# HipGraph/iSpLib

Measured on AMD Instinct MI355X. Metric: edges_aggregated_per_sec, higher is better.
Workload: dtype f32

## Files before the change

include/isplib_hip.h:

```cpp
#ifndef ISPLIB_HIP_H
#define ISPLIB_HIP_H

#include <stddef.h>
#include <stdint.h>

#ifdef __cplusplus
extern "C" {
#endif

#define ISPLIB_HIP_ABI_VERSION 1
#define ISPLIB_MAX_SLICES 4096

#define ISPLIB_VOP_COPY_RHS 0x2
#define ISPLIB_ROP_NOOP     0x00
#define ISPLIB_SOP_COPY     0x100
#define ISPLIB_VSC_MUL      0x1000
#define ISPLIB_VSC_MEAN     0x3000
#define ISPLIB_AOP_ADD      0x10000
#define ISPLIB_AOP_MAX      0x20000
#define ISPLIB_AOP_MIN      0x30000
#define ISPLIB_MSG_SPMM_SUM  (ISPLIB_VOP_COPY_RHS | ISPLIB_ROP_NOOP | ISPLIB_SOP_COPY | ISPLIB_VSC_MUL  | ISPLIB_AOP_ADD)
#define ISPLIB_MSG_SPMM_MEAN (ISPLIB_VOP_COPY_RHS | ISPLIB_ROP_NOOP | ISPLIB_SOP_COPY | ISPLIB_VSC_MEAN | ISPLIB_AOP_ADD)
#define ISPLIB_MSG_SPMM_MAX  (ISPLIB_VOP_COPY_RHS | ISPLIB_ROP_NOOP | ISPLIB_SOP_COPY | ISPLIB_VSC_MUL  | ISPLIB_AOP_MAX)
#define ISPLIB_MSG_SPMM_MIN  (ISPLIB_VOP_COPY_RHS | ISPLIB_ROP_NOOP | ISPLIB_SOP_COPY | ISPLIB_VSC_MUL  | ISPLIB_AOP_MIN)
// ... 133 lines not shown
typedef struct isplib_stream_plan {
   int64_t rows, cols;
   int32_t slices, gens, waves_per_gen, rows_per_wave, streams , chunk ;
   int64_t n_steps, n_parts, n_hub;
   const int32_t *words;
   const float   *vals;
   const int64_t *wave_step_off;
   const int32_t *wave_row;
   const int32_t *wave_part;
   const int32_t *hub_row;
   const int32_t *hub_off;
   const int32_t *perm;
} isplib_stream_plan;
int  isplib_stream_plan_build_hip(int64_t m, int64_t n, int64_t nnz, const int64_t *rowptr, const int64_t *col,
                                  const float *val, int streams, int slices, int chunk, int waves_per_gen,
                                  isplib_stream_plan *out , void *stream);
int  isplib_stream_plan_set_values_hip(isplib_stream_plan *plan, const float *val , void *stream);
void isplib_stream_plan_free(isplib_stream_plan *plan);
int    isplib_spmm_stream_geometry(int streams, int *rows_per_wave , int *waves_resident );
int    isplib_suggest_stream(int64_t m, int64_t n, int64_t nnz, int64_t k, int *streams, int *slices, int *chunk);
int    isplib_suggest_stream_weighted(int64_t m, int64_t n, int64_t nnz, int64_t k, int weighted, int *streams, int *slices, int *chunk);
int    isplib_spmm_stream_minmax_geometry(int streams , int *rows_per_wave , int *waves_resident );
int    isplib_suggest_stream_minmax(int64_t m, int64_t n, int64_t nnz, int64_t k, int *streams, int *slices, int *chunk);
int    isplib_stream_plan_build_minmax_hip(int64_t m, int64_t n, int64_t nnz, const int64_t *rowptr, const int64_t *col,
                                           const float *val, int streams, int slices, int chunk, int waves_per_gen,
                                           isplib_stream_plan *out , void *stream);
size_t isplib_spmm_stream_minmax_workspace_bytes(const isplib_stream_plan *plan);
int    fusedMM_csr_stream_minmax_hip(int32_t imessage , int64_t m, int64_t n, int64_t k,
                                     int64_t nnz, const int64_t *pntrb, const int64_t *pntre,
                                     const isplib_stream_plan *plan ,
                                     const float *y, int64_t ldy, float *z, int64_t ldz, int64_t *z_arg,
                                     void *workspace, size_t workspace_bytes, void *stream);
size_t isplib_spmm_stream_workspace_bytes(const isplib_stream_plan *plan);
int    fusedMM_csr_stream_hip(int32_t imessage , int64_t m, int64_t n, int64_t k,
                              int64_t nnz, const int64_t *pntrb, const int64_t *pntre,
                              const isplib_stream_plan *plan ,
                              const float *y, int64_t ldy, float *z, int64_t ldz,
                              void *workspace, size_t workspace_bytes,
                              const isplib_epilogue *epilogue , void *stream);

int    isplib_fusedmm_stream_geometry(int streams, int *rows_per_wave , int *waves_resident );
int    isplib_suggest_fusedmm_stream(int32_t imessage, int64_t m, int64_t n, int64_t nnz, int64_t k, int *streams, int *slices, int *chunk);
int    isplib_stream_plan_build_fusedmm_hip(int64_t m, int64_t n, int64_t nnz, const int64_t *rowptr, const int64_t *col,
                                            int streams, int slices, int chunk, int waves_per_gen,
                                            isplib_stream_plan *out , void *stream);
int    fusedMM_csr_udef_stream_hip(int32_t imessage, int64_t m, int64_t n, int64_t k, int64_t nnz,
                                   const int64_t *pntrb, const int64_t *pntre, const isplib_stream_plan *plan ,
                                   const float *x , int64_t ldx, const float *y , int64_t ldy,
                                   float *z , int64_t ldz, int sop_udef , float sop_param,
                                   void *workspace, size_t workspace_bytes, void *stream);

int    fusedMM_csr_ordered_hip(int32_t imessage, int64_t m, int64_t n, int64_t k, int64_t nnz, const float *val,
                               const int64_t *indx, const int64_t *pntrb, const int64_t *pntre,
                               const int32_t *row_order , const float *y, int64_t ldy, float *z,
                               int64_t ldz, int64_t *z_arg, void *stream);

int    isplib_plain_panels(int64_t n, int64_t ldy);

size_t isplib_community_order_workspace_bytes(int64_t m, int64_t nnz);
int    isplib_community_order_hip(int64_t m, int64_t nnz, const int64_t *rowptr, const int64_t *col, int rounds, int seed,
                                  int32_t *order, int32_t *labels , int *rounds_run ,
                                  void *workspace, size_t workspace_bytes, void *stream);
int    isplib_order_locality_hip(int64_t m, int64_t nnz, const int64_t *rowptr, const int64_t *col, const int32_t *order,
                                 int64_t window, double *share , void *workspace ,
                                 size_t workspace_bytes, void *stream);

// ... 64 lines not shown
```

isplib_amd/cabi.py:

```python
from __future__ import annotations

import ctypes
import os
from typing import Optional

import torch

from . import _lib

MSG_SPMM_SUM = 0x2 | 0x00 | 0x100 | 0x1000 | 0x10000
MSG_SPMM_MEAN = 0x2 | 0x00 | 0x100 | 0x3000 | 0x10000
MSG_SPMM_MAX = 0x2 | 0x00 | 0x100 | 0x1000 | 0x20000
MSG_SPMM_MIN = 0x2 | 0x00 | 0x100 | 0x1000 | 0x30000
MESSAGE = {"sum": MSG_SPMM_SUM, "add": MSG_SPMM_SUM, "mean": MSG_SPMM_MEAN, "max": MSG_SPMM_MAX, "min": MSG_SPMM_MIN}

SUCCESS, FAIL, NOT_ENOUGH_MEM, NO_OPT_IMPL, HIP_ERROR = 0, 1, -1, 128, 256
UNDEFINED_USER_FUNCTION = 64

VOP = {"copy_lhs": 0x1, "copy_rhs": 0x2, "add": 0x3, "subl": 0x4, "subr": 0x5, "max": 0x6, "min": 0x7, "udef": 0xF}
ROP = {"noop": 0x00, "dot": 0x10, "add_lhs": 0x20, "add_rhs": 0x30, "norml": 0x40, "normr": 0x50, "udef": 0xF0}
SOP = {"noop": 0x000, "copy": 0x100, "udef": 0xF00}
VSC = {"noop": 0x0000, "mul": 0x1000, "add": 0x2000, "mean": 0x3000, "udef": 0xF000}
AOP = {"add": 0x10000, "max": 0x20000, "min": 0x30000, "udef": 0xF0000}
SOP_UDEF = {"none": 0, "sigmoid": 1, "one_minus_sigmoid": 2, "tdist": 3, "scale": 4, "exp": 5, "leaky_exp": 6}
PATTERNS = {
    "spmm": (MSG_SPMM_SUM, "none"),
    "sigmoid_embedding": (VOP["copy_rhs"] | ROP["dot"] | SOP["udef"] | VSC["mul"] | AOP["add"], "sigmoid"),
    "tdist_embedding": (VOP["subr"] | ROP["normr"] | SOP["udef"] | VSC["mul"] | AOP["add"], "tdist"),
    "attention_sum": (VOP["copy_rhs"] | ROP["dot"] | SOP["udef"] | VSC["mul"] | AOP["add"], "leaky_exp"),
}

EXPORTS = (
    "isplib_hip_abi_version", "isplib_hip_last_error", "isplib_hip_set_empty_row", "isplib_hip_get_empty_row", "fusedMM_csr_hip", "performDummySpMM_hip",
    "isplib_spmm_minmax_bw_hip", "isplib_sddmm_csr_hip", "isplib_csr_row_ids_hip",
    "isplib_csr2csc_workspace_bytes", "isplib_csr2csc_hip",
    "isplib_spmm_slices_bytes", "isplib_spmm_slices_build_hip", "isplib_spmm_sliced_workspace_bytes",
    "fusedMM_csr_sliced_hip", "fusedMM_csr_sliced_phase_hip", "isplib_hip_tune",
    "isplib_spmm_tasks_workspace_bytes", "fusedMM_csr_tasks_hip",
    "isplib_spmm_tasks_plan_workspace_bytes", "isplib_spmm_tasks_count_hip", "isplib_spmm_tasks_fill_hip",
    "isplib_sddmm_csr_tasks_hip", "fusedMM_csr_tasks_epilogue_hip", "fusedMM_csr_udef_hip", "fusedMM_csr_udef_tasks_hip", "isplib_pack_indices_hip",
    "isplib_suggest_slices", "isplib_graph_create", "isplib_graph_set_slices", "isplib_graph_set_values", "isplib_graph_spmm", "isplib_graph_spmm_backward",
    "isplib_graph_destroy", "isplib_suggest_slices_whole_rows", "isplib_graph_sddmm",
    "fusedMM_csr_stream_hip", "isplib_spmm_stream_workspace_bytes", "isplib_spmm_stream_geometry", "isplib_suggest_stream", "isplib_suggest_stream_weighted", "isplib_stream_plan_build_hip", "isplib_stream_plan_build_minmax_hip", "fusedMM_csr_stream_minmax_hip", "isplib_spmm_stream_minmax_geometry", "isplib_suggest_stream_minmax", "isplib_spmm_stream_minmax_workspace_bytes", "isplib_stream_plan_set_values_hip", "isplib_stream_plan_free", "isplib_spmm_minmax_bw_det_hip", "isplib_spmm_minmax_bw_workspace_bytes", "isplib_scatter_rows_det_hip",
    "isplib_fusedmm_stream_geometry", "isplib_suggest_fusedmm_stream", "isplib_stream_plan_build_fusedmm_hip", "fusedMM_csr_udef_stream_hip",
    "isplib_row_scale_hip", "isplib_masked_scale_colsum_hip", "isplib_masked_scale_colsum_workspace_bytes",
    "fusedMM_csr_ordered_hip", "isplib_community_order_hip", "isplib_community_order_workspace_bytes", "isplib_order_locality_hip",
    "isplib_graph_set_row_order", "isplib_plain_panels",
)

EXP_EXPORTS = ("fusedMM_csr_sweep_hip", "isplib_spmm_sweep_workspace_bytes", "isplib_spmm_sweep_resident_waves",
               "fusedMM_csr_hybrid_hip", "isplib_spmm_hybrid_geometry", "isplib_spmm_hybrid_workspace_bytes", "isplib_sddmm_stream_hip",
               "isplib_hip_tune_experimental")

_i64, _f32, _vp, _i32 = ctypes.c_int64, ctypes.c_float, ctypes.c_void_p, ctypes.c_int32


class Epilogue(ctypes.Structure):
    _fields_ = [("row_scale", ctypes.c_void_p), ("self", ctypes.c_void_p), ("ld_self", ctypes.c_int64),
                ("bias", ctypes.c_void_p), ("relu", ctypes.c_int)]


class TaskPlanInfo(ctypes.Structure):
    _fields_ = [("n_tasks", ctypes.c_int64), ("lane_off", ctypes.c_int64 * 9), ("slices", ctypes.c_int32),
                ("chunk", ctypes.c_int32), ("short_row", ctypes.c_int32), ("reserved", ctypes.c_int32)]


class SweepPlanStruct(ctypes.Structure):
    _fields_ = [("rows", ctypes.c_int64), ("slices", ctypes.c_int32), ("gens", ctypes.c_int32),
                ("waves_per_gen", ctypes.c_int32), ("rows_per_wave", ctypes.c_int32), ("n_tasks", ctypes.c_int64),
                ("n_parts", ctypes.c_int64), ("n_hub", ctypes.c_int64), ("wave_row", ctypes.c_void_p),
                ("wave_part", ctypes.c_void_p), ("wave_task_off", ctypes.c_void_p), ("task_b", ctypes.c_void_p),
                ("task_meta", ctypes.c_void_p), ("hub_row", ctypes.c_void_p), ("hub_off", ctypes.c_void_p)]


class StreamPlanStruct(ctypes.Structure):
    _fields_ = [("rows", ctypes.c_int64), ("cols", ctypes.c_int64), ("slices", ctypes.c_int32), ("gens", ctypes.c_int32),
# ... 128 lines not shown
        L.isplib_spmm_stream_minmax_geometry.argtypes = [ctypes.c_int, ctypes.POINTER(ctypes.c_int), ctypes.POINTER(ctypes.c_int)]
        L.isplib_suggest_stream_minmax.restype = ctypes.c_int
        L.isplib_suggest_stream_minmax.argtypes = [_i64, _i64, _i64, _i64, ctypes.POINTER(ctypes.c_int), ctypes.POINTER(ctypes.c_int), ctypes.POINTER(ctypes.c_int)]
        L.isplib_spmm_stream_minmax_workspace_bytes.restype = ctypes.c_size_t
        L.isplib_spmm_stream_minmax_workspace_bytes.argtypes = [ctypes.POINTER(StreamPlanStruct)]
        L.fusedMM_csr_stream_minmax_hip.restype = ctypes.c_int
        L.fusedMM_csr_stream_minmax_hip.argtypes = [_i32, _i64, _i64, _i64, _i64, _vp, _vp, ctypes.POINTER(StreamPlanStruct), _vp, _i64,
                                                    _vp, _i64, _vp, _vp, ctypes.c_size_t, _vp]
        L.isplib_stream_plan_set_values_hip.restype = ctypes.c_int
        L.isplib_stream_plan_set_values_hip.argtypes = [ctypes.POINTER(StreamPlanStruct), _vp, _vp]
        L.isplib_stream_plan_free.restype = None
        L.isplib_stream_plan_free.argtypes = [ctypes.POINTER(StreamPlanStruct)]
        L.isplib_community_order_workspace_bytes.restype = ctypes.c_size_t
        L.isplib_community_order_workspace_bytes.argtypes = [_i64, _i64]
        L.isplib_community_order_hip.restype = ctypes.c_int
        L.isplib_community_order_hip.argtypes = [_i64, _i64, _vp, _vp, ctypes.c_int, ctypes.c_int, _vp, _vp, ctypes.POINTER(ctypes.c_int), _vp,
                                                 ctypes.c_size_t, _vp]
        L.isplib_order_locality_hip.restype = ctypes.c_int
        L.isplib_order_locality_hip.argtypes = [_i64, _i64, _vp, _vp, _vp, _i64, ctypes.POINTER(ctypes.c_double), _vp, ctypes.c_size_t, _vp]
        L.isplib_graph_set_row_order.restype = ctypes.c_int
        L.isplib_graph_set_row_order.argtypes = [_vp, _vp, _vp]
        L.fusedMM_csr_ordered_hip.restype = ctypes.c_int
        L.fusedMM_csr_ordered_hip.argtypes = [_i32, _i64, _i64, _i64, _i64, _vp, _vp, _vp, _vp, _vp, _vp, _i64, _vp, _i64, _vp, _vp]
        L.isplib_plain_panels.restype = ctypes.c_int
        L.isplib_plain_panels.argtypes = [_i64, _i64]
        L.isplib_suggest_stream.restype = ctypes.c_int
        L.isplib_suggest_stream.argtypes = [_i64, _i64, _i64, _i64, ctypes.POINTER(ctypes.c_int), ctypes.POINTER(ctypes.c_int), ctypes.POINTER(ctypes.c_int)]
        L.isplib_suggest_stream_weighted.restype = ctypes.c_int
        L.isplib_suggest_stream_weighted.argtypes = [_i64, _i64, _i64, _i64, ctypes.c_int, ctypes.POINTER(ctypes.c_int), ctypes.POINTER(ctypes.c_int), ctypes.POINTER(ctypes.c_int)]
        L.isplib_spmm_stream_geometry.restype = ctypes.c_int
        L.isplib_spmm_stream_geometry.argtypes = [ctypes.c_int, ctypes.POINTER(ctypes.c_int), ctypes.POINTER(ctypes.c_int)]
        L.isplib_spmm_stream_workspace_bytes.restype = ctypes.c_size_t
        L.isplib_spmm_stream_workspace_bytes.argtypes = [ctypes.POINTER(StreamPlanStruct)]
        L.fusedMM_csr_stream_hip.restype = ctypes.c_int
        L.fusedMM_csr_stream_hip.argtypes = [_i32, _i64, _i64, _i64, _i64, _vp, _vp, ctypes.POINTER(StreamPlanStruct), _vp, _i64,
                                             _vp, _i64, _vp, ctypes.c_size_t, ctypes.POINTER(Epilogue), _vp]
        _sigs_set = True
    return L


_exp = None


def exp_lib() -> ctypes.CDLL:
    global _exp
    if _exp is None:
        lib()
        path = os.path.join(os.path.dirname(_lib.CABI_PATH), "libisplib_hip_exp.so")
        if not os.path.exists(path):
            raise ImportError(f"isplib_amd: '{os.path.basename(path)}' not found; build it with `make -C isplib_amd/csrc`")
        L = ctypes.CDLL(path, mode=ctypes.RTLD_GLOBAL)
        L.isplib_hip_tune_experimental.restype = ctypes.c_int
        L.isplib_hip_tune_experimental.argtypes = [ctypes.c_int, ctypes.c_int]
        L.isplib_spmm_hybrid_geometry.restype = ctypes.c_int
        L.isplib_spmm_hybrid_geometry.argtypes = [ctypes.c_int] + [ctypes.POINTER(ctypes.c_int)] * 4
        L.isplib_spmm_hybrid_workspace_bytes.restype = ctypes.c_size_t
        L.isplib_spmm_hybrid_workspace_bytes.argtypes = [ctypes.POINTER(HybridPlanStruct)]
        L.fusedMM_csr_hybrid_hip.restype = ctypes.c_int
        L.fusedMM_csr_hybrid_hip.argtypes = [_i32, _i64, _i64, _i64, _i64, _vp, _vp, ctypes.POINTER(HybridPlanStruct), _vp, _i64, _vp, _i64,
                                             _vp, ctypes.c_size_t, _vp, _vp]
        L.isplib_sddmm_stream_hip.restype = ctypes.c_int
        L.isplib_sddmm_stream_hip.argtypes = [_i64, _i64, _i64, _i64, _vp, _vp, ctypes.POINTER(StreamPlanStruct), _vp, _i64, _vp, _i64,
                                              ctypes.c_int, _vp, _vp]
        L.isplib_spmm_sweep_resident_waves.restype = ctypes.c_int
        L.isplib_spmm_sweep_resident_waves.argtypes = [_i32, _i64, ctypes.c_int]
        L.isplib_spmm_sweep_workspace_bytes.restype = ctypes.c_size_t
# ... 585 lines not shown
        ep = Epilogue(None if row_scale is None else row_scale.data_ptr(), None if self_term is None else self_term.data_ptr(),
                      k if self_term is None else self_term.stride(0), None if bias is None else bias.data_ptr(), int(bool(relu)))
    fusedMM_csr_stream_hip(MESSAGE[reduce], rowptr, nnz, plan, y, out, workspace, ep)
    return out


def fusedMM_csr_stream_minmax_hip(imessage: int, rowptr, nnz: int, plan, y, z, z_arg=None, workspace=None, check: bool = True) -> int:
    assert y.is_cuda and y.dtype == torch.float32 and y.dim() == 2 and y.stride(1) == 1
    m, n, k = rowptr.numel() - 1, y.size(0), y.size(1)
    rp = rowptr.data_ptr()
    ps = plan.struct()
    with torch.cuda.device(y.device):
        st = lib().fusedMM_csr_stream_minmax_hip(int(imessage), m, n, k, int(nnz), ctypes.c_void_p(rp), ctypes.c_void_p(rp + 8),
                                                 ctypes.byref(ps), _ptr(y), y.stride(0) if n > 1 else max(k, y.stride(0)), _ptr(z),
                                                 z.stride(0) if m > 1 else max(k, z.stride(0)), _ptr(z_arg), _ptr(workspace),
                                                 0 if workspace is None else workspace.numel(), _stream(y.device))
    if check:
        _check(st, "fusedMM_csr_stream_minmax_hip")
    return st


def spmm_stream_minmax(rowptr, nnz: int, plan, y, reduce: str = "max", workspace=None, want_arg: bool = True):
    rowptr = _dev(rowptr, "rowptr", torch.int64)
    y = y.contiguous()
    m, k = rowptr.numel() - 1, y.size(1)
    out = torch.empty((m, k), dtype=torch.float32, device=y.device)
    arg = torch.empty((m, k), dtype=torch.int64, device=y.device) if want_arg else None
    if workspace is None:
        workspace = plan.workspace(minmax=True)
    fusedMM_csr_stream_minmax_hip(MESSAGE[reduce], rowptr, nnz, plan, y, out, arg, workspace)
    return out, arg


def suggest_stream_minmax(m: int, n: int, nnz: int, k: int):
    st, sl, ch = ctypes.c_int(0), ctypes.c_int(0), ctypes.c_int(0)
    if not lib().isplib_suggest_stream_minmax(int(m), int(n), int(nnz), int(k), ctypes.byref(st), ctypes.byref(sl), ctypes.byref(ch)):
        return None
    return st.value, sl.value, ch.value


def stream_minmax_geometry(streams: int = 4):
    rpw, res = ctypes.c_int(0), ctypes.c_int(0)
    _check(lib().isplib_spmm_stream_minmax_geometry(int(streams), ctypes.byref(rpw), ctypes.byref(res)), "isplib_spmm_stream_minmax_geometry")
    return rpw.value, res.value


def hybrid_geometry(streams: int = 4):
    v = [ctypes.c_int(0) for _ in range(4)]
    _check(exp_lib().isplib_spmm_hybrid_geometry(int(streams), *[ctypes.byref(x) for x in v]), "isplib_spmm_hybrid_geometry")
    return tuple(x.value for x in v)


def fusedMM_csr_hybrid_hip(imessage: int, rowptr, nnz: int, plan, y, z, workspace=None, epilogue=None, check: bool = True) -> int:
    assert y.is_cuda and y.dtype == torch.float32 and y.dim() == 2 and y.stride(1) == 1
    m, n, k = rowptr.numel() - 1, y.size(0), y.size(1)
    rp = rowptr.data_ptr()
    ps = plan.struct()
    with torch.cuda.device(y.device):
        st = exp_lib().fusedMM_csr_hybrid_hip(int(imessage), m, n, k, int(nnz), ctypes.c_void_p(rp), ctypes.c_void_p(rp + 8),
                                          ctypes.byref(ps), _ptr(y), y.stride(0) if n > 1 else max(k, y.stride(0)), _ptr(z),
                                          z.stride(0) if m > 1 else max(k, z.stride(0)), _ptr(workspace),
                                          0 if workspace is None else workspace.numel(),
                                          None if epilogue is None else ctypes.byref(epilogue), _stream(y.device))
    if check:
        _check(st, "fusedMM_csr_hybrid_hip")
    return st
# ... 179 lines not shown
```

isplib_amd/csrc/experimental/experimental.hip:

```cpp
#include "../sweep_common.h"
#include "../../../include/isplib_hip_experimental.h"

namespace isplib {

template <int OP, int LPR, int NVMAX> constexpr int sweep_lds_bytes() { return (OP == OP_ADD ? 1 : 2) * 4 * NVMAX * LPR * 4 * 4; }
template <int OP, int LPR, int NVMAX> constexpr int sweep_wgs_per_cu() {
   return 163840 / sweep_lds_bytes<OP, LPR, NVMAX>() < 8 ? 163840 / sweep_lds_bytes<OP, LPR, NVMAX>() : 8;
}

template <int OP, int LPR, int ADDR, int NVMAX>
__global__ __launch_bounds__(256, (sweep_wgs_per_cu<OP, LPR, NVMAX>())) void spmm_sweep_kernel(const SweepArgs a) {
   constexpr int VEC = 4, WAVES = 4, G = 64 / LPR, PANEL = LPR * VEC;
   constexpr int U = unroll_of<OP, 1, ADDR, true, LPR>();
   constexpr int PLANES = OP == OP_ADD ? 1 : 2;
   __shared__ __attribute__((aligned(16))) float s_all[PLANES * WAVES * NVMAX * PANEL];
   const int lane = threadIdx.x & 63;
   const int wave = __builtin_amdgcn_readfirstlane(threadIdx.x >> 6);
   const int g = lane / LPR, lc = lane % LPR;
   const int wl = (int)blockIdx.x * WAVES + wave;
   if (wl >= a.wave_count) return;
   const int64_t w = (int64_t)a.wave_base + wl;
   float *my_val = s_all + wave * (NVMAX * PANEL);
   int *my_idx = reinterpret_cast<int *>(s_all + WAVES * NVMAX * PANEL) + wave * (NVMAX * PANEL);
#pragma unroll
// ... 643 lines not shown
      p.ybytes = (unsigned)(yb - (unsigned long long)at * 4ull);
      for (int gen = 0; gen < plan->gens; gen++) {
         p.wave_base = gen * plan->waves_per_gen;
         p.wave_count = plan->waves_per_gen;
         int rc;
         if (plan->streams == 2) rc = first ? launch_sddmm_stream<32, false>(p, st) : launch_sddmm_stream<32, true>(p, st);
         else if (plan->streams == 4) rc = first ? launch_sddmm_stream<16, false>(p, st) : launch_sddmm_stream<16, true>(p, st);
         else rc = first ? launch_sddmm_stream<8, false>(p, st) : launch_sddmm_stream<8, true>(p, st);
         if (rc) return rc;
      }
      first = false;
   }
   return ISPLIB_SUCCESS;
}

struct HybridGeom { int nvmax, nbw, ht, hwr; };
static HybridGeom hybrid_geom(int streams) {
   if (streams == 8) return {ISPLIB_HYB8_NV, ISPLIB_HYB8_NBW, ISPLIB_HYB8_HT, ISPLIB_HYB8_HWR};
   return {ISPLIB_HYB4_NV, ISPLIB_HYB4_NBW, ISPLIB_HYB4_HT, ISPLIB_HYB4_HWR};
}

extern "C" int isplib_spmm_hybrid_geometry(int streams, int *rows_per_wave, int *waves_resident, int *table_rows, int *hot_cap) {
   clear_error();
   if (streams != 4 && streams != 8) return fail(ISPLIB_FAIL, "isplib_spmm_hybrid_geometry: streams must be 4 (64-column slots) or 8 (32-column slots)");
   const HybridGeom ge = hybrid_geom(streams);
   if (rows_per_wave) *rows_per_wave = ge.nvmax;
   if (waves_resident) *waves_resident = device_cus() * 8;
   if (table_rows) *table_rows = ge.ht;
   if (hot_cap) *hot_cap = ge.hwr * (64 / streams);
   return ISPLIB_SUCCESS;
}

extern "C" size_t isplib_spmm_hybrid_workspace_bytes(const isplib_hybrid_plan *plan) {
   return isplib_spmm_stream_workspace_bytes(plan ? &plan->cold : nullptr);
}

extern "C" int fusedMM_csr_hybrid_hip(int32_t imessage, int64_t m, int64_t n, int64_t k, int64_t nnz, const int64_t *pntrb,
                                      const int64_t *pntre, const isplib_hybrid_plan *hp, const float *y, int64_t ldy, float *z,
                                      int64_t ldz, void *workspace, size_t workspace_bytes, const isplib_epilogue *ep, void *stream) {
   clear_error();
   if (imessage != ISPLIB_MSG_SPMM_SUM && imessage != ISPLIB_MSG_SPMM_MEAN)
      return fail(ISPLIB_NO_OPT_IMPL, "fusedMM_csr_hybrid_hip: sum and mean only");
   if (m < 0 || n < 0 || k < 0 || nnz < 0) return fail(ISPLIB_FAIL, "fusedMM_csr_hybrid_hip: negative dimension");
   if (m == 0 || k == 0) return ISPLIB_SUCCESS;
   if (!hp) return fail(ISPLIB_FAIL, "fusedMM_csr_hybrid_hip: plan is required");
   const isplib_stream_plan *plan = &hp->cold;
   if (plan->rows != m || plan->cols != n) return fail(ISPLIB_FAIL, "fusedMM_csr_hybrid_hip: the plan was built for another shape");
   if (n >= (1LL << 24) || ldy >= (1LL << 22)) return fail(ISPLIB_FAIL, "fusedMM_csr_hybrid_hip: n must be < 2^24 and ldy < 2^22 (24-bit address arithmetic)");
   if (plan->streams != 4 && plan->streams != 8) return fail(ISPLIB_FAIL, "fusedMM_csr_hybrid_hip: bad plan geometry (streams 4 or 8)");
   const HybridGeom ge = hybrid_geom(plan->streams);
   if (plan->gens < 1 || plan->waves_per_gen < 8 || (plan->waves_per_gen % 8) != 0 || plan->rows_per_wave != ge.nvmax ||
       hp->table_rows != ge.ht || hp->hot_cap > ge.hwr * (64 / plan->streams) || plan->slices < 1)
      return fail(ISPLIB_FAIL, "fusedMM_csr_hybrid_hip: bad plan geometry (isplib_spmm_hybrid_geometry reports rows per wave, table rows and the hot-step cap; waves_per_gen must be a multiple of 8)");
   if (plan->vals) return fail(ISPLIB_FAIL, "fusedMM_csr_hybrid_hip: unit weights only (weighted graphs: fusedMM_csr_stream_hip)");
   if (k < 4) return fail(ISPLIB_FAIL, "fusedMM_csr_hybrid_hip: k >= 4 required (use fusedMM_csr_hip)");
   if (ldy < k || ldz < k) return fail(ISPLIB_FAIL, "fusedMM_csr_hybrid_hip: leading dimension smaller than k");
   const unsigned long long yb = (unsigned long long)n * (unsigned long long)ldy * 4ull;
   if (yb > BUF_LIMIT) return fail(ISPLIB_FAIL, "fusedMM_csr_hybrid_hip: dense operand larger than 3.5 GiB (use fusedMM_csr_hip)");
   if (!pntrb || !pntre || !z || !y || !plan->wave_row || !plan->wave_part || !plan->wave_step_off || (plan->n_steps > 0 && !plan->words) ||
       (plan->n_hub > 0 && (!plan->hub_row || !plan->hub_off)) || !hp->hot_rows || !hp->hot_step_off || (hp->n_hot_steps > 0 && !hp->hot_words))
      return fail(ISPLIB_FAIL, "fusedMM_csr_hybrid_hip: null operand");
   if (plan->n_parts > 0) {
      if (!workspace || workspace_bytes < isplib_spmm_stream_workspace_bytes(plan)) return fail(ISPLIB_NOT_ENOUGH_MEM, "fusedMM_csr_hybrid_hip: workspace too small");
      if (((uintptr_t)workspace & 255) != 0) return fail(ISPLIB_FAIL, "fusedMM_csr_hybrid_hip: workspace must be 256-byte aligned");
   }
   SweepArgs a = {};
   a.empty_init = empty_row_init();
   a.k = k; a.nnz = nnz; a.pntrb = pntrb; a.pntre = pntre;
   a.y = y; a.ldy = ldy; a.ybytes = (unsigned)yb; a.z = z; a.ldz = ldz;
   a.mean = imessage == ISPLIB_MSG_SPMM_MEAN ? 1 : 0;
   a.abs_ids = 1;
   a.wave_row = plan->wave_row; a.wave_part = plan->wave_part;
   a.words = plan->words; a.wave_step_off = plan->wave_step_off; a.null_word = (unsigned)n;
   a.hub_row = plan->hub_row; a.hub_off = plan->hub_off; a.n_hub = plan->n_hub;
   a.hot_rows = hp->hot_rows; a.hot_words = hp->hot_words; a.hot_step_off = hp->hot_step_off; a.slices = plan->slices;
   a.part_val = (float *)workspace;
   if (ep) {
      if (ep->self && ep->ld_self < k) return fail(ISPLIB_FAIL, "fusedMM_csr_hybrid_hip: ld_self smaller than k");
      a.ep_row_scale = ep->row_scale; a.ep_self = ep->self; a.ep_ld_self = ep->ld_self; a.ep_bias = ep->bias;
      a.ep_relu = ep->relu ? 1 : 0;
   }
   hipStream_t st = (hipStream_t)stream;
   const int64_t pw = 256 / plan->streams;
   for (int64_t c0 = 0; c0 < k; c0 += pw) {
      SweepArgs p = a;
      p.k = (k - c0) < pw ? (k - c0) : pw;
      if (p.k < 4) {
         p.k = 4;
         c0 = k - 4;
      }
      p.y = y + c0;
      p.z = z + c0;
      p.ep_self = a.ep_self ? a.ep_self + c0 : nullptr;
      p.ep_bias = a.ep_bias ? a.ep_bias + c0 : nullptr;
      p.ybytes = (unsigned)(yb - (unsigned long long)c0 * 4ull);
      for (int gen = 0; gen < plan->gens; gen++) {
// ... 31 lines not shown
```

isplib_amd/csrc/spmm_sweep.hip:

```cpp
#include "sweep_common.h"

namespace isplib {

template <int LPR, bool HAS_VAL, int NVMAX, int NBW, int WGS>
__global__ __launch_bounds__(256, (stream_wgs_per_cu<LPR, NVMAX, WGS>())) void spmm_stream_kernel(const SweepArgs a) {
   constexpr int WAVES = 4, G = 64 / LPR, PANEL = LPR * 4, U = 64 * NBW / G;
   constexpr int PER = NVMAX / G;
   constexpr int WAVE_FLOATS = NVMAX * PANEL;
   static_assert(NVMAX <= 256 && NVMAX % G == 0, "the local row is the top byte of a word");
   __shared__ __attribute__((aligned(16))) float s_all[WAVES * WAVE_FLOATS];
   const int lane = threadIdx.x & 63;
   const int wave = __builtin_amdgcn_readfirstlane(threadIdx.x >> 6);
   const int g = lane / LPR, lc = lane % LPR;
   const int wl = (int)blockIdx.x * WAVES + wave;
   if (wl >= a.wave_count) return;
   const int64_t w = (int64_t)a.wave_base + wl;
#ifdef ISPLIB_EXP_WAVE_TIMES
   const unsigned long long t_start = __builtin_amdgcn_s_memtime();
#endif
   float *my = s_all + wave * WAVE_FLOATS;
   for (int i = lane * 4; i < WAVE_FLOATS; i += 256)
      *reinterpret_cast<float4 *>(my + i) = make_float4(0.0f, 0.0f, 0.0f, 0.0f);
   __amdgpu_buffer_rsrc_t rsrc = __builtin_amdgcn_make_buffer_rsrc(const_cast<float *>(a.y), 0, (int)a.ybytes, 0x00020000);
   const bool cok = lc * 4 < a.k;
   int ccol = lc * 4, vfirst = 0;
   if (cok && ccol + 4 > (int)a.k) { vfirst = ccol + 4 - (int)a.k; ccol = (int)a.k - 4; }
   const unsigned cbyte = (unsigned)ccol * 4u, poison = cok ? 0u : BUF_OOB;
   float *lane_base = my + lc * 4;
   const int64_t s0 = a.wave_step_off[w], s1 = a.wave_step_off[w + 1];
   const int64_t nwords = (s1 - s0) * G;
   const int32_t *wp = a.words + s0 * G;
   const float *vp = HAS_VAL ? a.vals + s0 * G : nullptr;
   const unsigned ldyb = (unsigned)a.ldy * 4u;
// ... 356 lines not shown
   if (m <= 0 || n <= 0 || nnz <= 0 || k < 4 || n >= (1LL << 24) || nnz < (1LL << 22)) return 0;
   if (!stream_domain_ok(n, k, nnz)) return 0;
   int st = k <= 32 ? 8 : (k <= 64 ? 4 : (k < 128 ? 2 : 4));
   if (weighted && k >= 128 && (k % 128) == 0) st = 2;
   int rpw = 0, resident = 0;
   if (isplib_spmm_stream_geometry(st, &rpw, &resident) != ISPLIB_SUCCESS || rpw <= 0 || resident <= 0) return 0;
   if (!suggest_stream_geom(m, n, nnz, st, rpw, resident, 1.9e6, 3.4, slices, chunk)) {
      if (st != 2 || k < 128) return 0;
      st = 4;
      if (isplib_spmm_stream_geometry(st, &rpw, &resident) != ISPLIB_SUCCESS || rpw <= 0 || resident <= 0) return 0;
      if (!suggest_stream_geom(m, n, nnz, st, rpw, resident, 1.9e6, 3.4, slices, chunk)) return 0;
   }
   if (streams) *streams = st;
   return 1;
}

extern "C" int isplib_suggest_stream(int64_t m, int64_t n, int64_t nnz, int64_t k, int *streams, int *slices, int *chunk) {
   return isplib_suggest_stream_weighted(m, n, nnz, k, 0, streams, slices, chunk);
}

extern "C" int isplib_suggest_stream_minmax(int64_t m, int64_t n, int64_t nnz, int64_t k, int *streams, int *slices, int *chunk) {
   clear_error();
   if (m <= 0 || n <= 0 || nnz <= 0 || k < 4 || n >= (1LL << 24) || nnz < (1LL << 22) || nnz >= (1LL << 31)) return 0;
   if (!stream_domain_ok(n, k, nnz) || (unsigned long long)n * (unsigned long long)k * 4ull >= (1ull << 31)) return 0;
   const int st = k <= 32 ? 8 : 4;
   int rpw = 0, resident = 0;
   if (isplib_spmm_stream_minmax_geometry(st, &rpw, &resident) != ISPLIB_SUCCESS || rpw <= 0 || resident <= 0) return 0;
   if (!suggest_stream_geom(m, n, nnz, st, rpw, resident, 3.3e6, st == 8 ? 1.7 : 1.17, slices, chunk)) return 0;
   if (streams) *streams = st;
   return 1;
}

extern "C" size_t isplib_spmm_stream_workspace_bytes(const isplib_stream_plan *plan) {
   if (!plan || plan->n_parts <= 0) return 256;
   const size_t pk = (size_t)(256 / (plan->streams > 0 ? plan->streams : 4));
   return ((size_t)plan->n_parts * pk * sizeof(float) + 255) & ~(size_t)255;
}

extern "C" size_t isplib_spmm_stream_minmax_workspace_bytes(const isplib_stream_plan *plan) {
   return 2 * isplib_spmm_stream_workspace_bytes(plan);
}

static int stream_run(int32_t imessage, int64_t m, int64_t n, int64_t k, int64_t nnz, const int64_t *pntrb, const int64_t *pntre,
                      const isplib_stream_plan *plan, const float *y, int64_t ldy, float *z, int64_t ldz, int64_t *z_arg,
                      void *workspace, size_t workspace_bytes, const isplib_epilogue *ep, void *stream) {
   clear_error();
   const bool mm = imessage == ISPLIB_MSG_SPMM_MAX || imessage == ISPLIB_MSG_SPMM_MIN;
   if (imessage != ISPLIB_MSG_SPMM_SUM && imessage != ISPLIB_MSG_SPMM_MEAN && !mm)
      return fail(ISPLIB_NO_OPT_IMPL, "fusedMM_csr_stream_hip: message outside the SpMM set");
   if (m < 0 || n < 0 || k < 0 || nnz < 0) return fail(ISPLIB_FAIL, "fusedMM_csr_stream_hip: negative dimension");
   if (m == 0 || k == 0) return ISPLIB_SUCCESS;
   if (!plan) return fail(ISPLIB_FAIL, "fusedMM_csr_stream_hip: plan is required");
   if (plan->rows != m || plan->cols != n) return fail(ISPLIB_FAIL, "fusedMM_csr_stream_hip: the plan was built for another shape");
   if (n >= (1LL << 24) || ldy >= (1LL << 22)) return fail(ISPLIB_FAIL, "fusedMM_csr_stream_hip: n must be < 2^24 and ldy < 2^22 (24-bit address arithmetic)");
   if (plan->streams != 2 && plan->streams != 4 && plan->streams != 8)
      return fail(ISPLIB_FAIL, "fusedMM_csr_stream_hip: bad plan geometry (streams 2, 4 or 8)");
   if (mm && plan->streams != 4 && plan->streams != 8) return fail(ISPLIB_FAIL, "fusedMM_csr_stream_hip: max / min run on 4- or 8-stream plans (isplib_spmm_stream_minmax_geometry)");
   if (plan->gens < 1 || plan->waves_per_gen < 1 || plan->rows_per_wave != stream_geom(plan->streams, mm).nvmax)
      return fail(ISPLIB_FAIL, "fusedMM_csr_stream_hip: bad plan geometry (rows_per_wave must be what isplib_spmm_stream_geometry / _minmax_geometry reports)");
   if (mm && plan->n_steps > 0 && !plan->perm) return fail(ISPLIB_FAIL, "fusedMM_csr_stream_hip: max / min need the plan's perm array (the winners' CSR positions)");
   if (mm && nnz >= (1LL << 31)) return fail(ISPLIB_FAIL, "fusedMM_csr_stream_hip: max / min need nnz < 2^31");
   if (mm && ep) return fail(ISPLIB_FAIL, "fusedMM_csr_stream_hip: the epilogue is defined for sum / mean only");
   if (mm && (unsigned long long)n * (unsigned long long)ldy * 4ull >= (1ull << 31))
      return fail(ISPLIB_FAIL, "fusedMM_csr_stream_minmax_hip: dense operand of 2 GiB or more (use fusedMM_csr_tasks_hip)");
   if (k < 4) return fail(ISPLIB_FAIL, "fusedMM_csr_stream_hip: k >= 4 required (use fusedMM_csr_hip)");
   if (ldy < k || ldz < k) return fail(ISPLIB_FAIL, "fusedMM_csr_stream_hip: leading dimension smaller than k");
   const unsigned long long yb = (unsigned long long)n * (unsigned long long)ldy * 4ull;
   if (yb > BUF_LIMIT) return fail(ISPLIB_FAIL, "fusedMM_csr_stream_hip: dense operand larger than 3.5 GiB (use fusedMM_csr_hip)");
   if (!pntrb || !pntre || !z || !y || !plan->wave_row || !plan->wave_part || !plan->wave_step_off ||
       (plan->n_steps > 0 && !plan->words) || (plan->n_hub > 0 && (!plan->hub_row || !plan->hub_off)))
      return fail(ISPLIB_FAIL, "fusedMM_csr_stream_hip: null operand");
   if (plan->n_parts > 0) {
      if (!workspace || workspace_bytes < (mm ? 2 : 1) * isplib_spmm_stream_workspace_bytes(plan)) return fail(ISPLIB_NOT_ENOUGH_MEM, "fusedMM_csr_stream_hip: workspace too small");
      if (((uintptr_t)workspace & 255) != 0) return fail(ISPLIB_FAIL, "fusedMM_csr_stream_hip: workspace must be 256-byte aligned");
   }
   SweepArgs a = {};
   a.empty_init = empty_row_init();
   a.k = k; a.nnz = nnz; a.pntrb = pntrb; a.pntre = pntre;
   a.y = y; a.ldy = ldy; a.ybytes = (unsigned)yb; a.z = z; a.ldz = ldz; a.z_arg = z_arg;
   a.mean = imessage == ISPLIB_MSG_SPMM_MEAN ? 1 : 0;
   a.ids = plan->perm; a.abs_ids = 1;
   a.wave_row = plan->wave_row; a.wave_part = plan->wave_part;
   a.words = plan->words; a.vals = plan->vals; a.wave_step_off = plan->wave_step_off; a.null_word = (unsigned)n;
   a.hub_row = plan->hub_row; a.hub_off = plan->hub_off; a.n_hub = plan->n_hub;
   a.part_val = (float *)workspace;
   a.part_idx = mm && workspace ? (int *)((char *)workspace + isplib_spmm_stream_workspace_bytes(plan)) : nullptr;
   if (ep) {
      if (ep->self && ep->ld_self < k) return fail(ISPLIB_FAIL, "fusedMM_csr_stream_hip: ld_self smaller than k");
      a.ep_row_scale = ep->row_scale; a.ep_self = ep->self; a.ep_ld_self = ep->ld_self; a.ep_bias = ep->bias;
      a.ep_relu = ep->relu ? 1 : 0;
   }
   hipStream_t st = (hipStream_t)stream;
   const int64_t pw = 256 / plan->streams;
   for (int64_t c0 = 0; c0 < k; c0 += pw) {
      SweepArgs p = a;
      p.k = (k - c0) < pw ? (k - c0) : pw;
      if (p.k < 4) {
         p.k = 4;
         c0 = k - 4;
      }
      p.y = y + c0;
      p.z = z + c0;
      p.ep_self = a.ep_self ? a.ep_self + c0 : nullptr;
      p.ep_bias = a.ep_bias ? a.ep_bias + c0 : nullptr;
      p.z_arg = z_arg ? z_arg + c0 : nullptr;
      p.ybytes = (unsigned)(yb - (unsigned long long)c0 * 4ull);
      for (int gen = 0; gen < plan->gens; gen++) {
         p.wave_base = gen * plan->waves_per_gen;
         p.wave_count = plan->waves_per_gen;
         int rc;
         if (imessage == ISPLIB_MSG_SPMM_MAX) rc = plan->vals ? launch_stream_minmax<OP_MAX, true>(p, st, plan->streams) : launch_stream_minmax<OP_MAX, false>(p, st, plan->streams);
         else if (imessage == ISPLIB_MSG_SPMM_MIN) rc = plan->vals ? launch_stream_minmax<OP_MIN, true>(p, st, plan->streams) : launch_stream_minmax<OP_MIN, false>(p, st, plan->streams);
         else if (plan->streams == 2) rc = plan->vals ? launch_stream<32, true>(p, st) : launch_stream<32, false>(p, st);
         else if (plan->streams == 4) rc = plan->vals ? launch_stream<16, true>(p, st) : launch_stream<16, false>(p, st);
         else rc = plan->vals ? launch_stream<8, true>(p, st) : launch_stream<8, false>(p, st);
         if (rc) return rc;
      }
      if (plan->n_hub > 0) {
         const bool v4 = (p.k % 4) == 0 && (p.ldz % 4) == 0 && ((uintptr_t)p.z & 15) == 0 && (!p.ep_self || ((p.ep_ld_self % 4) == 0 && ((uintptr_t)p.ep_self & 15) == 0));
         int64_t blocks = (plan->n_hub * (v4 ? p.k / 4 : p.k) + 255) / 256;
         if (blocks > 4096) blocks = 4096;
         if (imessage == ISPLIB_MSG_SPMM_MAX) {
            if (v4) hipLaunchKernelGGL((sweep_hub_fold_kernel<OP_MAX, 4>), dim3((unsigned)blocks), dim3(256), 0, st, p);
            else hipLaunchKernelGGL((sweep_hub_fold_kernel<OP_MAX, 1>), dim3((unsigned)blocks), dim3(256), 0, st, p);
         } else if (imessage == ISPLIB_MSG_SPMM_MIN) {
            if (v4) hipLaunchKernelGGL((sweep_hub_fold_kernel<OP_MIN, 4>), dim3((unsigned)blocks), dim3(256), 0, st, p);
            else hipLaunchKernelGGL((sweep_hub_fold_kernel<OP_MIN, 1>), dim3((unsigned)blocks), dim3(256), 0, st, p);
         } else if (v4) hipLaunchKernelGGL((sweep_hub_fold_kernel<OP_ADD, 4>), dim3((unsigned)blocks), dim3(256), 0, st, p);
         else hipLaunchKernelGGL((sweep_hub_fold_kernel<OP_ADD, 1>), dim3((unsigned)blocks), dim3(256), 0, st, p);
         const int rc = check_launch("sweep_hub_fold_kernel");
         if (rc) return rc;
      }
   }
   return ISPLIB_SUCCESS;
}

extern "C" int fusedMM_csr_stream_hip(int32_t imessage, int64_t m, int64_t n, int64_t k, int64_t nnz,
                                      const int64_t *pntrb, const int64_t *pntre, const isplib_stream_plan *plan,
                                      const float *y, int64_t ldy, float *z, int64_t ldz, void *workspace,
// ... 23 lines not shown
```

Measured before the change: 42.62 billion.

## Stage dense panel into padded workspace to avoid slow cache-line slot

Adds a cost model that counts how many 128-byte lines of each dense-operand column panel fall into a particular address slot within a 1 KiB period, treated as slow. When the estimated penalty outweighs the cost of a copy, the panel is copied into a workspace region with a 64- or 128-float pitch before the streaming SpMM kernels run, and those kernels then read the staged copy. Workspace size grows to hold the staged panel, and the hybrid path is switched to the partial-only size. This adds an extra copy kernel and more workspace memory, and it relies on a hardware address-slot assumption that may not hold.

```diff
diff --git a/include/isplib_hip.h b/include/isplib_hip.h
--- a/include/isplib_hip.h
+++ b/include/isplib_hip.h
@@ -189,6 +189,9 @@
                                      const float *y, int64_t ldy, float *z, int64_t ldz, int64_t *z_arg,
                                      void *workspace, size_t workspace_bytes, void *stream);
 size_t isplib_spmm_stream_workspace_bytes(const isplib_stream_plan *plan);
+size_t isplib_spmm_stream_partial_bytes(const isplib_stream_plan *plan);
+int    isplib_stream_bad_line_share(uintptr_t y, int64_t ldy, int64_t c0, int64_t cols, int64_t *bad_lines , int64_t *lines );
+int    isplib_stream_stage_place(uintptr_t workspace, size_t used_bytes, int64_t cols, uintptr_t *base , int64_t *pitch );
 int    fusedMM_csr_stream_hip(int32_t imessage , int64_t m, int64_t n, int64_t k,
                               int64_t nnz, const int64_t *pntrb, const int64_t *pntre,
                               const isplib_stream_plan *plan ,
diff --git a/isplib_amd/cabi.py b/isplib_amd/cabi.py
--- a/isplib_amd/cabi.py
+++ b/isplib_amd/cabi.py
@@ -41,7 +41,7 @@
     "isplib_sddmm_csr_tasks_hip", "fusedMM_csr_tasks_epilogue_hip", "fusedMM_csr_udef_hip", "fusedMM_csr_udef_tasks_hip", "isplib_pack_indices_hip",
     "isplib_suggest_slices", "isplib_graph_create", "isplib_graph_set_slices", "isplib_graph_set_values", "isplib_graph_spmm", "isplib_graph_spmm_backward",
     "isplib_graph_destroy", "isplib_suggest_slices_whole_rows", "isplib_graph_sddmm",
-    "fusedMM_csr_stream_hip", "isplib_spmm_stream_workspace_bytes", "isplib_spmm_stream_geometry", "isplib_suggest_stream", "isplib_suggest_stream_weighted", "isplib_stream_plan_build_hip", "isplib_stream_plan_build_minmax_hip", "fusedMM_csr_stream_minmax_hip", "isplib_spmm_stream_minmax_geometry", "isplib_suggest_stream_minmax", "isplib_spmm_stream_minmax_workspace_bytes", "isplib_stream_plan_set_values_hip", "isplib_stream_plan_free", "isplib_spmm_minmax_bw_det_hip", "isplib_spmm_minmax_bw_workspace_bytes", "isplib_scatter_rows_det_hip",
+    "fusedMM_csr_stream_hip", "isplib_spmm_stream_workspace_bytes", "isplib_spmm_stream_partial_bytes", "isplib_stream_bad_line_share", "isplib_stream_stage_place", "isplib_spmm_stream_geometry", "isplib_suggest_stream", "isplib_suggest_stream_weighted", "isplib_stream_plan_build_hip", "isplib_stream_plan_build_minmax_hip", "fusedMM_csr_stream_minmax_hip", "isplib_spmm_stream_minmax_geometry", "isplib_suggest_stream_minmax", "isplib_spmm_stream_minmax_workspace_bytes", "isplib_stream_plan_set_values_hip", "isplib_stream_plan_free", "isplib_spmm_minmax_bw_det_hip", "isplib_spmm_minmax_bw_workspace_bytes", "isplib_scatter_rows_det_hip",
     "isplib_fusedmm_stream_geometry", "isplib_suggest_fusedmm_stream", "isplib_stream_plan_build_fusedmm_hip", "fusedMM_csr_udef_stream_hip",
     "isplib_row_scale_hip", "isplib_masked_scale_colsum_hip", "isplib_masked_scale_colsum_workspace_bytes",
     "fusedMM_csr_ordered_hip", "isplib_community_order_hip", "isplib_community_order_workspace_bytes", "isplib_order_locality_hip",
@@ -236,6 +236,12 @@
         L.isplib_spmm_stream_geometry.argtypes = [ctypes.c_int, ctypes.POINTER(ctypes.c_int), ctypes.POINTER(ctypes.c_int)]
         L.isplib_spmm_stream_workspace_bytes.restype = ctypes.c_size_t
         L.isplib_spmm_stream_workspace_bytes.argtypes = [ctypes.POINTER(StreamPlanStruct)]
+        L.isplib_spmm_stream_partial_bytes.restype = ctypes.c_size_t
+        L.isplib_spmm_stream_partial_bytes.argtypes = [ctypes.POINTER(StreamPlanStruct)]
+        L.isplib_stream_bad_line_share.restype = ctypes.c_int
+        L.isplib_stream_bad_line_share.argtypes = [ctypes.c_size_t, _i64, _i64, _i64, ctypes.POINTER(_i64), ctypes.POINTER(_i64)]
+        L.isplib_stream_stage_place.restype = ctypes.c_int
+        L.isplib_stream_stage_place.argtypes = [ctypes.c_size_t, ctypes.c_size_t, _i64, ctypes.POINTER(ctypes.c_size_t), ctypes.POINTER(_i64)]
         L.fusedMM_csr_stream_hip.restype = ctypes.c_int
         L.fusedMM_csr_stream_hip.argtypes = [_i32, _i64, _i64, _i64, _i64, _vp, _vp, ctypes.POINTER(StreamPlanStruct), _vp, _i64,
                                              _vp, _i64, _vp, ctypes.c_size_t, ctypes.POINTER(Epilogue), _vp]
@@ -887,6 +893,20 @@
     return out, arg
 
 
+def stream_bad_line_share(y_addr: int, ldy: int, c0: int, cols: int):
+    bad, total = _i64(0), _i64(0)
+    _check(lib().isplib_stream_bad_line_share(int(y_addr), int(ldy), int(c0), int(cols), ctypes.byref(bad), ctypes.byref(total)),
+           "isplib_stream_bad_line_share")
+    return bad.value, total.value
+
+
+def stream_stage_place(workspace_addr: int, used_bytes: int, cols: int):
+    base, pitch = ctypes.c_size_t(0), _i64(0)
+    _check(lib().isplib_stream_stage_place(int(workspace_addr), int(used_bytes), int(cols), ctypes.byref(base), ctypes.byref(pitch)),
+           "isplib_stream_stage_place")
+    return base.value, pitch.value
+
+
 def suggest_stream_minmax(m: int, n: int, nnz: int, k: int):
     st, sl, ch = ctypes.c_int(0), ctypes.c_int(0), ctypes.c_int(0)
     if not lib().isplib_suggest_stream_minmax(int(m), int(n), int(nnz), int(k), ctypes.byref(st), ctypes.byref(sl), ctypes.byref(ch)):
diff --git a/isplib_amd/csrc/experimental/experimental.hip b/isplib_amd/csrc/experimental/experimental.hip
--- a/isplib_amd/csrc/experimental/experimental.hip
+++ b/isplib_amd/csrc/experimental/experimental.hip
@@ -699,7 +699,7 @@
 }
 
 extern "C" size_t isplib_spmm_hybrid_workspace_bytes(const isplib_hybrid_plan *plan) {
-   return isplib_spmm_stream_workspace_bytes(plan ? &plan->cold : nullptr);
+   return isplib_spmm_stream_partial_bytes(plan ? &plan->cold : nullptr);
 }
 
 extern "C" int fusedMM_csr_hybrid_hip(int32_t imessage, int64_t m, int64_t n, int64_t k, int64_t nnz, const int64_t *pntrb,
@@ -728,7 +728,7 @@
        (plan->n_hub > 0 && (!plan->hub_row || !plan->hub_off)) || !hp->hot_rows || !hp->hot_step_off || (hp->n_hot_steps > 0 && !hp->hot_words))
       return fail(ISPLIB_FAIL, "fusedMM_csr_hybrid_hip: null operand");
    if (plan->n_parts > 0) {
-      if (!workspace || workspace_bytes < isplib_spmm_stream_workspace_bytes(plan)) return fail(ISPLIB_NOT_ENOUGH_MEM, "fusedMM_csr_hybrid_hip: workspace too small");
+      if (!workspace || workspace_bytes < isplib_spmm_stream_partial_bytes(plan)) return fail(ISPLIB_NOT_ENOUGH_MEM, "fusedMM_csr_hybrid_hip: workspace too small");
       if (((uintptr_t)workspace & 255) != 0) return fail(ISPLIB_FAIL, "fusedMM_csr_hybrid_hip: workspace must be 256-byte aligned");
    }
    SweepArgs a = {};
diff --git a/isplib_amd/csrc/line_slots.h b/isplib_amd/csrc/line_slots.h
--- /dev/null
+++ b/isplib_amd/csrc/line_slots.h
@@ -0,0 +1,64 @@
+#pragma once
+#include <stddef.h>
+#include <stdint.h>
+
+#include "../../include/isplib_hip.h"
+
+namespace isplib {
+
+constexpr unsigned LINE_SLOW_SLOT = 3;
+
+constexpr double STAGE_PENALTY_PS = 1.7;
+constexpr double STAGE_COPY_BYTES_PER_PS = 4.2;
+#ifndef ISPLIB_STAGE_MARGIN
+#define ISPLIB_STAGE_MARGIN 2.0
+#endif
+constexpr double STAGE_MARGIN = ISPLIB_STAGE_MARGIN;
+constexpr size_t STAGE_CAP_BYTES = (size_t)1 << 30;
+
+static inline void line_slot_count(uintptr_t base, int64_t pitch, int64_t first, int64_t width, int64_t *bad, int64_t *total, int64_t *rows) {
+   int64_t step = pitch % 1024, period = 1;
+   if (step < 0) step += 1024;
+   if (step != 0) {
+      int64_t a = step, b = 1024;
+      while (b) { const int64_t t = a % b; a = b; b = t; }
+      period = 1024 / a;
+   }
+   const uint64_t b0 = ((uint64_t)base + (uint64_t)first) & 1023u;
+   int64_t nb = 0, nt = 0;
+   if (width > 0)
+      for (int64_t r = 0; r < period; r++) {
+         const uint64_t lo = (b0 + (uint64_t)(r * step)) & 1023u, hi = lo + (uint64_t)width - 1;
+         for (uint64_t line = lo >> 7; line <= hi >> 7; line++) {
+            nt++;
+            if ((line & 7u) == LINE_SLOW_SLOT) nb++;
+         }
+      }
+   *bad = nb; *total = nt; *rows = period;
+}
+
+static inline int64_t stage_pitch_floats(int64_t cols) { return cols == 32 ? 64 : (cols == 64 ? 128 : 0); }
+
+static inline size_t stream_partial_bytes(const isplib_stream_plan *plan) {
+   if (!plan || plan->n_parts <= 0) return 256;
+   const size_t pk = (size_t)(256 / (plan->streams > 0 ? plan->streams : 4));
+   return ((size_t)plan->n_parts * pk * sizeof(float) + 255) & ~(size_t)255;
+}
+
+static inline bool stage_pays(double words, double bad_per_row, double n, double panel_bytes) {
+   return words * bad_per_row * STAGE_PENALTY_PS > STAGE_MARGIN * n * panel_bytes * 2.0 / STAGE_COPY_BYTES_PER_PS;
+}
+
+static inline size_t stream_stage_bytes(const isplib_stream_plan *plan) {
+   if (!plan || plan->cols <= 0 || plan->n_steps <= 0 || (plan->streams != 4 && plan->streams != 8)) return 0;
+   const int64_t pw = 256 / plan->streams, pitch = stage_pitch_floats(pw);
+   if ((double)plan->cols * (double)pitch * 4.0 >= (double)STAGE_CAP_BYTES) return 0;
+   if (!stage_pays((double)plan->n_steps * plan->streams, (double)pw * 4.0 / 128.0, (double)plan->cols, (double)pw * 4.0)) return 0;
+   return 1024 + (size_t)plan->cols * (size_t)pitch * sizeof(float);
+}
+
+static inline uintptr_t stage_base(uintptr_t workspace, size_t used) { return (workspace + used + 1023) & ~(uintptr_t)1023; }
+
+int stage_panel(int64_t n, const float *src, int64_t lds, float *dst, int64_t ldd, int64_t cols, void *stream);
+
+}
diff --git a/isplib_amd/csrc/spmm_sweep.hip b/isplib_amd/csrc/spmm_sweep.hip
--- a/isplib_amd/csrc/spmm_sweep.hip
+++ b/isplib_amd/csrc/spmm_sweep.hip
@@ -1,4 +1,5 @@
 #include "sweep_common.h"
+#include "line_slots.h"
 
 namespace isplib {
 
@@ -421,13 +422,11 @@
 }
 
 extern "C" size_t isplib_spmm_stream_workspace_bytes(const isplib_stream_plan *plan) {
-   if (!plan || plan->n_parts <= 0) return 256;
-   const size_t pk = (size_t)(256 / (plan->streams > 0 ? plan->streams : 4));
-   return ((size_t)plan->n_parts * pk * sizeof(float) + 255) & ~(size_t)255;
+   return stream_partial_bytes(plan) + stream_stage_bytes(plan);
 }
 
 extern "C" size_t isplib_spmm_stream_minmax_workspace_bytes(const isplib_stream_plan *plan) {
-   return 2 * isplib_spmm_stream_workspace_bytes(plan);
+   return 2 * stream_partial_bytes(plan) + stream_stage_bytes(plan);
 }
 
 static int stream_run(int32_t imessage, int64_t m, int64_t n, int64_t k, int64_t nnz, const int64_t *pntrb, const int64_t *pntre,
@@ -460,7 +459,7 @@
        (plan->n_steps > 0 && !plan->words) || (plan->n_hub > 0 && (!plan->hub_row || !plan->hub_off)))
       return fail(ISPLIB_FAIL, "fusedMM_csr_stream_hip: null operand");
    if (plan->n_parts > 0) {
-      if (!workspace || workspace_bytes < (mm ? 2 : 1) * isplib_spmm_stream_workspace_bytes(plan)) return fail(ISPLIB_NOT_ENOUGH_MEM, "fusedMM_csr_stream_hip: workspace too small");
+      if (!workspace || workspace_bytes < (mm ? 2 : 1) * stream_partial_bytes(plan)) return fail(ISPLIB_NOT_ENOUGH_MEM, "fusedMM_csr_stream_hip: workspace too small");
       if (((uintptr_t)workspace & 255) != 0) return fail(ISPLIB_FAIL, "fusedMM_csr_stream_hip: workspace must be 256-byte aligned");
    }
    SweepArgs a = {};
@@ -473,7 +472,7 @@
    a.words = plan->words; a.vals = plan->vals; a.wave_step_off = plan->wave_step_off; a.null_word = (unsigned)n;
    a.hub_row = plan->hub_row; a.hub_off = plan->hub_off; a.n_hub = plan->n_hub;
    a.part_val = (float *)workspace;
-   a.part_idx = mm && workspace ? (int *)((char *)workspace + isplib_spmm_stream_workspace_bytes(plan)) : nullptr;
+   a.part_idx = mm && workspace ? (int *)((char *)workspace + stream_partial_bytes(plan)) : nullptr;
    if (ep) {
       if (ep->self && ep->ld_self < k) return fail(ISPLIB_FAIL, "fusedMM_csr_stream_hip: ld_self smaller than k");
       a.ep_row_scale = ep->row_scale; a.ep_self = ep->self; a.ep_ld_self = ep->ld_self; a.ep_bias = ep->bias;
@@ -481,6 +480,12 @@
    }
    hipStream_t st = (hipStream_t)stream;
    const int64_t pw = 256 / plan->streams;
+   float *stage = nullptr;
+   size_t stage_room = 0;
+   if (workspace) {
+      const uintptr_t w0 = (uintptr_t)workspace, sb = stage_base(w0, (mm ? 2 : 1) * stream_partial_bytes(plan));
+      if (sb < w0 + workspace_bytes) { stage = (float *)sb; stage_room = (size_t)(w0 + workspace_bytes - sb); }
+   }
    for (int64_t c0 = 0; c0 < k; c0 += pw) {
       SweepArgs p = a;
       p.k = (k - c0) < pw ? (k - c0) : pw;
@@ -494,6 +499,17 @@
       p.ep_bias = a.ep_bias ? a.ep_bias + c0 : nullptr;
       p.z_arg = z_arg ? z_arg + c0 : nullptr;
       p.ybytes = (unsigned)(yb - (unsigned long long)c0 * 4ull);
+      const int64_t sp = stage_pitch_floats(p.k);
+      if (stage && sp > 0 && (ldy % 4) == 0 && ((uintptr_t)p.y & 15) == 0 && (size_t)n * (size_t)sp * sizeof(float) <= stage_room &&
+          (size_t)n * (size_t)sp * sizeof(float) < STAGE_CAP_BYTES) {
+         int64_t bad = 0, total = 0, rows = 0;
+         line_slot_count((uintptr_t)y, ldy * 4, c0 * 4, p.k * 4, &bad, &total, &rows);
+         if (bad > 0 && stage_pays((double)plan->n_steps * plan->streams, (double)bad / (double)rows, (double)n, (double)p.k * 4.0)) {
+            const int rc = stage_panel(n, p.y, ldy, stage, sp, p.k, stream);
+            if (rc) return rc;
+            p.y = stage; p.ldy = sp; p.ybytes = (unsigned)((unsigned long long)n * (unsigned long long)sp * 4ull);
+         }
+      }
       for (int gen = 0; gen < plan->gens; gen++) {
          p.wave_base = gen * plan->waves_per_gen;
          p.wave_count = plan->waves_per_gen;
diff --git a/isplib_amd/csrc/stage_panel.hip b/isplib_amd/csrc/stage_panel.hip
--- /dev/null
+++ b/isplib_amd/csrc/stage_panel.hip
@@ -0,0 +1,61 @@
+#include <hip/hip_runtime.h>
+#include <stdint.h>
+
+#include "../../include/isplib_hip.h"
+#include "common.h"
+#include "line_slots.h"
+
+namespace isplib {
+
+__global__ __launch_bounds__(256) void stage_panel_kernel(int64_t n, const float *__restrict__ src, int64_t lds, float *__restrict__ dst,
+                                                          int64_t ldd, int vshift) {
+   const int64_t total = n << vshift, stride = (int64_t)gridDim.x * 256;
+   const int64_t vmask = ((int64_t)1 << vshift) - 1;
+   for (int64_t i = (int64_t)blockIdx.x * 256 + threadIdx.x; i < total; i += 4 * stride) {
+      float4 v[4];
+#pragma unroll
+      for (int q = 0; q < 4; q++) {
+         const int64_t j = i + q * stride;
+         if (j < total) v[q] = *reinterpret_cast<const float4 *>(src + (j >> vshift) * lds + (j & vmask) * 4);
+      }
+#pragma unroll
+      for (int q = 0; q < 4; q++) {
+         const int64_t j = i + q * stride;
+         if (j < total) *reinterpret_cast<float4 *>(dst + (j >> vshift) * ldd + (j & vmask) * 4) = v[q];
+      }
+   }
+}
+
+int stage_panel(int64_t n, const float *src, int64_t lds, float *dst, int64_t ldd, int64_t cols, void *stream) {
+   if (n <= 0) return ISPLIB_SUCCESS;
+   if ((cols != 32 && cols != 64) || lds < cols || ldd < cols || (lds % 4) != 0 || (ldd % 4) != 0 || (((uintptr_t)src | (uintptr_t)dst) & 15) != 0)
+      return fail(ISPLIB_FAIL, "stage_panel: 32 or 64 columns of 16-byte aligned rows");
+   const int vshift = cols == 32 ? 3 : 4;
+   int64_t blocks = ((n << vshift) + 1023) / 1024;
+   if (blocks > 65536) blocks = 65536;
+   hipLaunchKernelGGL(stage_panel_kernel, dim3((unsigned)blocks), dim3(256), 0, (hipStream_t)stream, n, src, lds, dst, ldd, vshift);
+   return check_launch("stage_panel_kernel");
+}
+
+}
+
+using namespace isplib;
+
+extern "C" int isplib_stream_bad_line_share(uintptr_t y, int64_t ldy, int64_t c0, int64_t cols, int64_t *bad_lines, int64_t *lines) {
+   clear_error();
+   if (ldy <= 0 || c0 < 0 || cols <= 0) return fail(ISPLIB_FAIL, "isplib_stream_bad_line_share: ldy and cols must be positive, c0 not negative");
+   int64_t bad = 0, total = 0, rows = 0;
+   line_slot_count(y, ldy * 4, c0 * 4, cols * 4, &bad, &total, &rows);
+   if (bad_lines) *bad_lines = bad;
+   if (lines) *lines = total;
+   return ISPLIB_SUCCESS;
+}
+
+extern "C" size_t isplib_spmm_stream_partial_bytes(const isplib_stream_plan *plan) { return stream_partial_bytes(plan); }
+
+extern "C" int isplib_stream_stage_place(uintptr_t workspace, size_t used_bytes, int64_t cols, uintptr_t *base, int64_t *pitch) {
+   clear_error();
+   if (base) *base = stage_base(workspace, used_bytes);
+   if (pitch) *pitch = stage_pitch_floats(cols);
+   return ISPLIB_SUCCESS;
+}
```

After: 45.09 billion (median of 6 runs). 1.06x the previous value.
